# Ajax0564/VyomAI

Hardware: AMD Instinct MI355X
Metric: training tokens/sec (12L d=768 seq=512 GPT-style decoder, CLM) (higher is better)
Workload: dtype bf16; 1 GPU; configs[1]: GPT-style Decoder 12L d=768 h=12 RoPE vocab 50265, CLM training B=32/GPU seq=512, AdamW, bf16 kernels + fp32 masters; global_batch=32, seq_len=512, parallelism=dp1, attention=none, weights=deterministic recipe (vyomai_amd.recipe)

## Files before the change

### include/vyom_hip.h

```cpp
#ifndef VYOM_HIP_H
#define VYOM_HIP_H

#include <stdint.h>

#ifdef __cplusplus
extern "C" {
#endif

typedef enum { VY_F32 = 0, VY_BF16 = 1 } vy_dtype;

typedef enum {
  VY_OK = 0,
  VY_ERR_ARG = -1,
  VY_ERR_UNSUPPORTED = -2,
  VY_ERR_LAUNCH = -3
} vy_status;

typedef enum {
  VY_ACT_NONE = 0, VY_ACT_GELU_ERF = 1, VY_ACT_GELU_TANH = 2,
  VY_ACT_SILU = 3, VY_ACT_TANH = 4, VY_ACT_SIGMOID = 5, VY_ACT_RELU6 = 6, VY_ACT_LEAKY_RELU = 7
} vy_act;
#define VY_ACT_SAVE_DERIV 0x100

enum {
// ... 71 lines not shown
int vy_gated_act_fwd(const void* gate_up, int64_t ldg, void* out, int64_t ldo, int64_t M, int64_t I,
                     int act, int dtype, void* stream);

int vy_rmsnorm_bwd(const void* dy, int64_t lddy, const void* x, int64_t ldx, const void* w,
                   const void* add_to, int64_t ldadd, void* dx, int64_t lddx, float* dw, float beta,
                   float* ws, int64_t M, int64_t N, float eps, float w_offset, int dtype, void* stream);

int vy_gated_act_bwd(const void* d_act, int64_t lddo, const void* gate_up, int64_t ldg, void* d_gate_up,
                     int64_t lddg, int64_t M, int64_t I, int act, int dtype, void* stream);

int vy_rope_fwd(void* x, int64_t sb, int64_t sh, int64_t sl, const float* cos_tab,
                const float* sin_tab, int64_t pos0, int64_t B, int heads, int64_t L, int dh,
                int inverse, int dtype, void* stream);


int vy_linear_dgrad(const void* dy, int64_t lddy, const void* wt, int64_t ldwt, const void* pre,
                    int64_t ldpre, int act, const void* add_to, int64_t ldadd, const void* add_to2,
                    int64_t ldadd2, void* dx, int64_t lddx, int64_t M, int64_t N, int64_t K, int dtype,
                    void* stream);

int vy_linear_wgrad(const void* dy, int64_t lddy, const void* x, int64_t ldx, float* dw,
                    int64_t lddw, float* db, float beta, const float* alpha_dev, int64_t M, int64_t N,
                    int64_t K, int dtype, void* stream);

typedef struct vy_wgrad_desc {
  const void* dy; int64_t lddy;
  const void* x; int64_t ldx;
  float* dw; int64_t lddw;
  float* db;
  int64_t M, N, K;
} vy_wgrad_desc;
int vy_linear_wgrad_grouped(const vy_wgrad_desc* descs, int32_t n, int dtype, void* stream);

typedef struct vy_colsum_desc {
  float* ws; int32_t W, N;
  float* out0; float* out1;
  int32_t acc;
} vy_colsum_desc;
int vy_linear_wgrad_grouped_cs(const vy_wgrad_desc* descs, int32_t n, const vy_colsum_desc* cs, int32_t ncs, int dtype,
                               void* stream);

int64_t vy_layernorm_bwd_ws_rows(int64_t M);
int vy_layernorm_bwd(const void* dy, int64_t lddy, const void* x, int64_t ldx, const void* gamma,
                     const float* mean, const float* rstd, void* dx, int64_t lddx, float* dgamma,
                     float* dbeta, float beta, float* ws, int64_t M, int64_t N, int dtype,
                     void* stream);
// ... 26 lines not shown
                  float grad_scale, const float* grad_scale_dev, void* stream);
int vy_adamw_step_gated(float* p, const float* g, float* m, float* v, void* p_bf16, int64_t n, float lr,
                        float beta1, float beta2, float eps, float weight_decay, int64_t step,
                        float grad_scale, const float* grad_scale_dev, const float* gate, void* stream);

int vy_sumsq(const float* x, int64_t n, float* out, float* ws, void* stream);

int vy_linear_dropout_fwd(const void* x, int64_t ldx, const void* w, int64_t ldw, const void* bias,
                          const void* residual, int64_t ldr, void* y, int64_t ldy, int64_t M, int64_t N,
                          int64_t K, float p_drop, uint64_t seed, uint64_t offset, int dtype, void* stream);
int vy_dropout(const void* x, int64_t ldx, void* y, int64_t ldy, int64_t M, int64_t N, float p_drop,
               uint64_t seed, uint64_t offset, int dtype, void* stream);

int vy_act_bwd(const void* dy, int64_t lddy, const void* pre, int64_t ldpre, void* dx, int64_t lddx,
               int64_t M, int64_t N, int act, int dtype, void* stream);

int vy_xent_fwd(const void* logits, int64_t ld, const int64_t* labels, int64_t ignore_index, float* lse,
                float* loss_sum, float* count, int64_t M, int64_t V, int32_t* err_flag, int dtype, void* stream);
int vy_xent_bwd(void* logits, int64_t ld, const int64_t* labels, int64_t ignore_index, const float* lse,
                const float* gscale, const float* count, int64_t M, int64_t V, int dtype, void* stream);
int vy_xent_fused(void* logits, int64_t ld, const int64_t* labels, int64_t ignore_index, float* lse,
                  float* loss_sum, const float* count, const float* gscale, int64_t M, int64_t V,
                  int32_t* err_flag, int dtype, void* stream);
int vy_xent_sample_fwd(const void* logits, int64_t ld, const int64_t* labels, int64_t ignore_index, float* lse,
                       float* loss_sum, float* count, int64_t* sampled, float inv_temperature, uint64_t seed,
                       uint64_t offset, int64_t M, int64_t V, int32_t* err_flag, int dtype, void* stream);
int vy_xent_sample_fused(void* logits, int64_t ld, const int64_t* labels, int64_t ignore_index, float* lse,
                         float* loss_sum, const float* count, const float* gscale, int64_t* sampled,
                         float inv_temperature, uint64_t seed, uint64_t offset, int64_t M, int64_t V,
                         int32_t* err_flag, int dtype, void* stream);
int vy_gumbel_noise(float* out, int64_t ld, int64_t M, int64_t V, uint64_t seed, uint64_t offset, void* stream);

int vy_bce_head_fwd(const void* h, int64_t ldh, const void* w, const void* b, float* z, const float* target,
                    const uint8_t* live, float* loss_sum, int64_t M, int64_t d, int dtype, void* stream);
int vy_bce_head_bwd(const void* h, int64_t ldh, const void* w, const float* z, const float* target,
                    const uint8_t* live, const float* gscale, const float* count, void* dh, int64_t lddh, float* dw,
                    float* db, int accumulate, int64_t M, int64_t d, int dtype, void* stream);

int vy_mlm_mask(const int64_t* ids, int64_t n, const int64_t* special_ids, int32_t n_special, float fraction,
                int64_t mask_id, int64_t vocab, int64_t ignore_index, uint64_t seed, uint64_t offset,
                int64_t* masked_ids, int64_t* labels, uint8_t* masked, void* stream);


int vy_logprob_fwd(const void* logits, int64_t ld, const int64_t* labels, const float* weight, float* lse,
                   float* logp, int64_t M, int64_t V, int32_t* err_flag, int dtype, void* stream);
int vy_logprob_bwd(void* logits, int64_t ld, const int64_t* labels, const float* weight, const float* lse,
// ... 81 lines not shown
```

### vyomai_amd/_lib.py

```python
from __future__ import annotations

import ctypes as C
import os
from typing import Optional

_HERE = os.path.dirname(os.path.abspath(__file__))
LIB_PATH = os.environ.get("VY_LIB_PATH") or os.path.join(_HERE, "lib", "libvyom_hip.so")

VY_F32, VY_BF16 = 0, 1
ACT_NONE, ACT_GELU_ERF, ACT_GELU_TANH = 0, 1, 2
ACT_SILU, ACT_TANH, ACT_SIGMOID, ACT_RELU6, ACT_LEAKY_RELU = 3, 4, 5, 6, 7
ACT_SAVE_DERIV = 0x100
MASK_NONE, MASK_CAUSAL, MASK_KEYPAD, MASK_ADDITIVE = 0, 1, 2, 4

_p, _i64, _i, _f, _u64 = C.c_void_p, C.c_int64, C.c_int, C.c_float, C.c_uint64

PROTOTYPES = {
    "vy_linear_fwd": [_p, _i64, _p, _i64, _p, _p, _i64, _p, _i64, _p, _i64, _i64, _i64, _i, _i, _p],
    "vy_qkv_rope_fwd": [_p, _i64, _p, _i64, _p, _p, _p, _i64,
                        _p, _i64, _i64, _i64, _p, _i64, _i64, _i64, _p, _i64, _i64, _i64,
                        _i64, _i64, _i64, _i, _i, _i, _i, _p],
    "vy_attn_fwd": [_p, _i64, _i64, _i64, _p, _i64, _i64, _i64, _p, _i64, _i64, _i64,
                    _p, _i64, _i64, _p, _i, _i64, _p, _i64, _p, _i64, _i64,
                    _i64, _i, _i, _i64, _i64, _i, _f, _i, _p],
    "vy_attn_decode": [_p, _i64, _i64, _p, _i64, _i64, _i64, _p, _i64, _i64, _i64,
                       _p, _i64, _i64, _i, _i, _i64, _i, _f, _i, _p],
    "vy_paged_rope_write": [_p, _i64, _p, _p, _p, _p, _i64, _p, _p, _i64, _i, _i64, _i, _i, _i, _i, _p],
    "vy_paged_qknorm_rope_write": [_p, _i64, _p, _p, _p, _p, _i64, _p, _p, _f, _p, _p, _i64, _i, _i64, _i, _i, _i, _i,
                                   _p],
    "vy_attn_paged_decode": [_p, _i64, _p, _p, _p, _i64, _i, _p, _i64, _p, _i64, _p, _i64, _i64, _i, _i, _i, _f, _i,
                             _p, _i64, _i, _p],
    "vy_attn_paged_prefill": [_p, _i64, _p, _p, _i64, _i, _p, _i64, _p, _p, _i64, _i64, _i64, _p, _i64, _i, _i, _i, _f,
                              _i, _p],
    "vy_paged_gather": [_p, _p, _i64, _i, _p, _i64, _i64, _p, _p, _i, _i, _i, _p],
    "vy_layernorm_fwd": [_p, _i64, _p, _p, _p, _i64, _p, _p, _i64, _i64, _f, _i, _p],
    "vy_rmsnorm_fwd": [_p, _i64, _p, _p, _i64, _i64, _i64, _f, _f, _i, _p],
    "vy_gated_act_fwd": [_p, _i64, _p, _i64, _i64, _i64, _i, _i, _p],
    "vy_rmsnorm_bwd": [_p, _i64, _p, _i64, _p, _p, _i64, _p, _i64, _p, _f, _p, _i64, _i64, _f, _f, _i, _p],
    "vy_gated_act_bwd": [_p, _i64, _p, _i64, _p, _i64, _i64, _i64, _i, _i, _p],
    "vy_rope_fwd": [_p, _i64, _i64, _i64, _p, _p, _i64, _i64, _i, _i64, _i, _i, _i, _p],
    "vy_linear_dgrad": [_p, _i64, _p, _i64, _p, _i64, _i, _p, _i64, _p, _i64, _p, _i64, _i64, _i64, _i64, _i, _p],
    "vy_linear_wgrad": [_p, _i64, _p, _i64, _p, _i64, _p, _f, _p, _i64, _i64, _i64, _i, _p],
    "vy_linear_wgrad_grouped": [_p, _i, _i, _p],
    "vy_linear_wgrad_grouped_cs": [_p, _i, _p, _i, _i, _p],
    "vy_layernorm_bwd_partial": [_p, _i64, _p, _i64, _p, _p, _p, _p, _i64, _p, _i64, _i64, _i, _p],
    "vy_layernorm_bwd": [_p, _i64, _p, _i64, _p, _p, _p, _p, _i64, _p, _p, _f, _p, _i64, _i64, _i, _p],
    "vy_attn_bwd": [_p, _i64, _i64, _i64, _p, _i64, _i64, _i64, _p, _i64, _i64, _i64,
                    _p, _p, _i64, _i64, _p, _p,
                    _p, _i64, _i64, _i64, _p, _i64, _i64, _i64, _p, _i64, _i64, _i64,
                    _i, _i64, _p, _i64, _p, _p, _i64, _i64, _i, _i, _i64, _i64, _i, _f, _i, _p],
    "vy_adamw_step": [_p, _p, _p, _p, _p, _i64, _f, _f, _f, _f, _f, _i64, _f, _p, _p],
    "vy_adamw_step_gated": [_p, _p, _p, _p, _p, _i64, _f, _f, _f, _f, _f, _i64, _f, _p, _p, _p],
    "vy_sumsq": [_p, _i64, _p, _p, _p],
    "vy_linear_dropout_fwd": [_p, _i64, _p, _i64, _p, _p, _i64, _p, _i64, _i64, _i64, _i64, _f, _u64, _u64, _i, _p],
    "vy_dropout": [_p, _i64, _p, _i64, _i64, _i64, _f, _u64, _u64, _i, _p],
    "vy_act_bwd": [_p, _i64, _p, _i64, _p, _i64, _i64, _i64, _i, _i, _p],
    "vy_xent_fwd": [_p, _i64, _p, _i64, _p, _p, _p, _i64, _i64, _p, _i, _p],
    "vy_xent_bwd": [_p, _i64, _p, _i64, _p, _p, _p, _i64, _i64, _i, _p],
    "vy_xent_fused": [_p, _i64, _p, _i64, _p, _p, _p, _p, _i64, _i64, _p, _i, _p],
    "vy_xent_sample_fwd": [_p, _i64, _p, _i64, _p, _p, _p, _p, _f, _u64, _u64, _i64, _i64, _p, _i, _p],
    "vy_xent_sample_fused": [_p, _i64, _p, _i64, _p, _p, _p, _p, _p, _f, _u64, _u64, _i64, _i64, _p, _i, _p],
    "vy_gumbel_noise": [_p, _i64, _i64, _i64, _u64, _u64, _p],
    "vy_bce_head_fwd": [_p, _i64, _p, _p, _p, _p, _p, _p, _i64, _i64, _i, _p],
    "vy_bce_head_bwd": [_p, _i64, _p, _p, _p, _p, _p, _p, _p, _i64, _p, _p, _i, _i64, _i64, _i, _p],
    "vy_mlm_mask": [_p, _i64, _p, _i, _f, _i64, _i64, _i64, _u64, _u64, _p, _p, _p, _p],
    "vy_logprob_fwd": [_p, _i64, _p, _p, _p, _p, _i64, _i64, _p, _i, _p],
    "vy_logprob_bwd": [_p, _i64, _p, _p, _p, _i64, _i64, _i, _p],
    "vy_logprob_fused": [_p, _i64, _p, _p, _p, _p, _i64, _i64, _p, _i, _p],
    "vy_transpose_batched": [_p, _i, _i, _i, _p],
    "vy_embedding_fwd": [_p, _i64, _p, _p, _i64, _i64, _i64, _i64, _p, _i, _p],
    "vy_embedding_bwd": [_p, _i64, _p, _p, _i64, _i64, _i64, _i64, _i64, _i, _p],
    "vy_transpose": [_p, _i64, _p, _i64, _i64, _i64, _i, _p],
    "vy_greedy_step": [_p, _i64, _i64, _i64, _i, _p, _i64, _i64, _p, _i64, _p, _i, _p, _p, _p],
    "vy_sampling_probs": [_p, _i64, _i64, _i64, _i, _f, _i, _f, _p, _i64, _p],
    "vy_sample_rows": [_p, _i64, _i64, _i64, _i, _p, _p, _p, _p, _p, _p, _p],
    "vy_decoder_step": [_p, _p, _i64, _p, _p, _p, _i64, _p],
    "vy_gemma_decoder_step": [_p, _p, _i64, _p, _i64, _p],
    "vy_cast": [_p, _p, _i64, _i, _i, _p],
    "vy_ddp_unique_id": [_p],
    "vy_ddp_init": [_p, _i, _i],
    "vy_ddp_all_reduce_async": [_p, _i64, _i, _p],
    "vy_ddp_destroy": [],
# ... 67 lines not shown
```

### vyomai_amd/autograd_train.py

```python
from __future__ import annotations

import os

import weakref
from typing import Optional

import torch

from . import _lib, ops
from ._lib import ACT_GELU_ERF, ACT_NONE, VyomHipError
from .layers.attention import _shadow
from .layers.mask import AttnMask
from .layers.positional_embeddings import resolve_freqs

BF16 = torch.bfloat16


WEIGHT_EPOCH = [0]


class _WtRegistry:

    def __init__(self) -> None:
        self.entries = []
# ... 523 lines not shown
    logits = buf[:, :V]
    ops.linear(n.view(buf.shape[0], -1), _shadow(w, dt), None if bias is None else _shadow(bias, dt), out=logits)
    return buf, logits


def _rehome(x, ld, dtype, reuse=False):
    V = x.shape[-1]
    if reuse and x.stride(-1) == 1 and x.stride(-2) == ld and x.dtype == dtype:
        buf = torch.as_strided(x, (*x.shape[:-1], ld), x.stride())
        if ld != V:
            buf[..., V:].zero_()
        return buf
    buf = torch.zeros((*x.shape[:-1], ld), dtype=dtype, device=x.device)
    buf[..., :V] = x
    return buf


def _shifted_labels(labels, ignore_index, dev):
    shifted = torch.full(labels.shape, ignore_index, dtype=torch.long, device=dev)
    shifted[:, :-1] = labels[:, 1:]
    return shifted.view(-1)


def _xent_forward(logits, shifted, ignore_index, err_flag=None, in_place=True, sample=None):
    V = logits.shape[1]
    dev = logits.device
    lse = torch.empty(logits.shape[0], dtype=torch.float32, device=dev)
    acc = torch.zeros(2, dtype=torch.float32, device=dev)
    fused = in_place and V <= 65536 and logits.dtype == BF16
    if fused:
        acc[1] = ((shifted != ignore_index) & (shifted >= 0) & (shifted < V)).sum()
        if sample is None:
            ops.xent_fused_(logits, shifted, ignore_index, lse, acc[0:1], acc[1:2], _one(dev), err_flag)
        else:
            ops.xent_sample_fused_(logits, shifted, ignore_index, lse, acc[0:1], acc[1:2], _one(dev), *sample, err_flag)
    elif sample is None:
        ops.xent_fwd(logits, shifted, ignore_index, lse, acc[0:1], acc[1:2], err_flag)
    else:
        ops.xent_sample_fwd(logits, shifted, ignore_index, lse, acc[0:1], acc[1:2], *sample, err_flag)
    return acc[0] / acc[1].clamp_min(1.0), lse, acc, fused


def _xent_backward(logits, shifted, ignore_index, lse, acc, fused, gout):
    gs = gout.detach().to(torch.float32).reshape(1).contiguous()
    if fused:
        return gs
    ops.xent_bwd_(logits, shifted, ignore_index, lse, gs, acc[1:2])
    return None


class LMHeadFn(torch.autograd.Function):

    @staticmethod
    def forward(ctx, hidden, wd, bd, ln_w, ln_b, wv, bias, eps):
        _require_bf16(hidden)
        dt = hidden.dtype
        pre, g, n, mean, rstd = _head_transform(hidden, wd, bd, ln_w, ln_b, eps)
        V = wv.shape[0]
        ld = _row_stride(V)
        buf = torch.zeros((*hidden.shape[:-1], ld), dtype=dt, device=hidden.device)
        logits = buf[..., :V]
        ops.linear(n, _shadow(wv, dt), _shadow(bias, dt), out=logits)
        ctx.save_for_backward(hidden, pre, g, n, mean, rstd)
        ctx.params = (wd, bd, ln_w, ln_b, wv, bias)
        ctx.ld = ld
        return logits

    @staticmethod
    def backward(ctx, dlogits):
        hidden, pre, g, n, mean, rstd = ctx.saved_tensors
        wd, bd, ln_w, ln_b, wv, bias = ctx.params
        dt = hidden.dtype
        buf = _rehome(dlogits, ctx.ld, dt, reuse=True)
        dn = ops.linear_dgrad(buf, _wt_padded(wv, dt, ctx.ld))
        dwv, dbias = _wgrad(buf[..., :wv.shape[0]], n, wv, bias)
        return (*_head_transform_backward(dn, hidden, pre, g, mean, rstd, wd, bd, ln_w, ln_b), dwv, dbias, None)


class LMHeadLossFn(torch.autograd.Function):

    @staticmethod
    def forward(ctx, hidden, labels, ignore_index, wd, bd, ln_w, ln_b, wv, bias, eps, err_flag=None, shift=True,
                sample=None):
        _require_bf16(hidden)
        pre, g, n, mean, rstd = _head_transform(hidden, wd, bd, ln_w, ln_b, eps)
        buf, logits = _vocab_logits(n, wv, bias)
        dev = hidden.device
        shifted = _shifted_labels(labels, ignore_index, dev) if shift else labels.to(dev).reshape(-1).contiguous()
        sampled = None
        if sample is not None:
            sampled = torch.empty(shifted.shape, dtype=torch.long, device=dev)
            sample = (sampled, *sample)
        loss, lse, acc, fused = _xent_forward(logits, shifted, ignore_index, err_flag, sample=sample)
        ctx.save_for_backward(hidden, pre, g, n, mean, rstd, buf, shifted, lse, acc)
        ctx.params = (wd, bd, ln_w, ln_b, wv, bias)
        ctx.ignore = ignore_index
        ctx.fused = fused
        if sampled is None:
            return loss
        sampled = sampled.view(labels.shape)
        ctx.mark_non_differentiable(sampled)
        return loss, sampled

    @staticmethod
    def backward(ctx, gout, *_):
        hidden, pre, g, n, mean, rstd, buf, shifted, lse, acc = ctx.saved_tensors
        wd, bd, ln_w, ln_b, wv, bias = ctx.params
        dt = hidden.dtype
        logits = buf[:, :wv.shape[0]]
        alpha = _xent_backward(logits, shifted, ctx.ignore, lse, acc, ctx.fused, gout)
        dn = ops.linear_dgrad(buf, _wt_padded(wv, dt, buf.shape[1]))
        if alpha is not None:
            dn = dn * alpha.to(dt)
        dwv, dbias = _wgrad(logits, n.view(buf.shape[0], -1), wv, bias, alpha=alpha)
        dh, dwd, dbd, dgam, dbet = _head_transform_backward(dn.view(g.shape), hidden, pre, g, mean, rstd, wd, bd, ln_w, ln_b)
        return dh, None, None, dwd, dbd, dgam, dbet, dwv, dbias, None, None, None, None
# ... 256 lines not shown
        ctx.save_for_backward(n)
        ctx.meta = (table, table_pending, ld)
        return logits

    @staticmethod
    def backward(ctx, dlogits):
        (n,) = ctx.saved_tensors
        table, table_pending, ld = ctx.meta
        V = table.shape[0]
        buf = _rehome(dlogits.reshape(-1, V), ld, n.dtype)
        dn, dtab = _tied_head_backward(buf, V, n, table, table_pending, None)
        return dn, dtab, None


class ShiftedXentFn(torch.autograd.Function):

    @staticmethod
    def forward(ctx, logits, labels, ignore_index):
        _require_bf16(logits)
        B, L, V = logits.shape
        if logits.stride(-1) != 1 or logits.stride(1) % 8 or logits.stride(0) != L * logits.stride(1):
            logits = _rehome(logits, _row_stride(V), logits.dtype)[..., :V]
        l2 = torch.as_strided(logits, (B * L, V), (logits.stride(1), 1), logits.storage_offset())
        shifted = _shifted_labels(labels, ignore_index, logits.device)
        loss, lse, acc, _ = _xent_forward(l2, shifted, ignore_index, in_place=False)
        ctx.save_for_backward(l2, shifted, lse, acc)
        ctx.meta = (ignore_index, (B, L, V))
        return loss

    @staticmethod
    def backward(ctx, gout):
        l2, shifted, lse, acc = ctx.saved_tensors
        ignore_index, shape = ctx.meta
        ld = l2.stride(0)
        buf = torch.empty((l2.shape[0], ld), dtype=l2.dtype, device=l2.device)
        d2 = buf[:, :l2.shape[1]]
        d2.copy_(l2)
        _xent_backward(d2, shifted, ignore_index, lse, acc, False, gout)
        return torch.as_strided(buf, shape, (shape[1] * ld, ld, 1)), None, None


class TiedLMHeadLossFn(torch.autograd.Function):

    @staticmethod
    def forward(ctx, hidden, labels, ignore_index, ln_w, eps, table, table_pending, err_flag=None):
        _require_bf16(hidden)
        n = ops.rmsnorm(hidden, _shadow(ln_w, hidden.dtype), eps, 0.0)
        buf, logits = _vocab_logits(n, table, None)
        shifted = _shifted_labels(labels, ignore_index, hidden.device)
        loss, lse, acc, fused = _xent_forward(logits, shifted, ignore_index, err_flag)
        ctx.save_for_backward(hidden, n, buf, shifted, lse, acc)
        ctx.meta = (ln_w, eps, table, table_pending, ignore_index, fused)
        return loss

    @staticmethod
    def backward(ctx, gout):
        hidden, n, buf, shifted, lse, acc = ctx.saved_tensors
        ln_w, eps, table, table_pending, ignore_index, fused = ctx.meta
        V = table.shape[0]
        alpha = _xent_backward(buf[:, :V], shifted, ignore_index, lse, acc, fused, gout)
        dn, dtab = _tied_head_backward(buf, V, n, table, table_pending, alpha)
        dh, dlnw = _rms_bwd(dn, hidden, ln_w, eps)
        return dh, None, None, dlnw, None, dtab, None, None


def logprob_rows(input_ids, selection_mask):
    B, L = input_ids.shape
    labels = torch.zeros((B, L), dtype=torch.long, device=input_ids.device)
    labels[:, :-1] = input_ids[:, 1:]
    m = selection_mask.to(device=input_ids.device, dtype=torch.float32)
    w = torch.zeros((B, L), dtype=torch.float32, device=input_ids.device)
    w[:, :-1] = m[:, 1:]
    total = w.sum(-1, keepdim=True)
# ... 41 lines not shown
```

### vyomai_amd/csrc/vy_bwd.hip

```cpp
#include "vy_attn_tile.h"
#include <float.h>
#include <stdlib.h>
#include <string.h>

namespace {


__device__ __forceinline__ int xcd_remap(int bid, int nwg) {
  const int xcd = bid & 7, q = nwg >> 3, r = nwg & 7;
  return (xcd < r ? xcd * (q + 1) : r * (q + 1) + (xcd - r) * q) + (bid >> 3);
}

__device__ __forceinline__ bf16x8 tr_pair(const char* base, int row_bytes) {
  const s16x4 lo = __builtin_amdgcn_ds_read_tr16_b64_v4i16((VY_LDS s16x4*)(base));
  const s16x4 hi = __builtin_amdgcn_ds_read_tr16_b64_v4i16((VY_LDS s16x4*)(base + 8 * row_bytes));
  union { struct { s16x4 a, b; } s; bf16x8 v; } u;
  u.s.a = lo; u.s.b = hi;
  return u.v;
}

typedef __attribute__((ext_vector_type(2))) __bf16 bf16x2_t;

template <int BT, int MS_, bool MF16>
struct WgradTile {
// ... 231 lines not shown
    }
    const bool hi = kq >= 2;
#pragma unroll
    for (int i = 0; i < TI; ++i)
#pragma unroll
      for (int jp = 0; jp < JH; ++jp) {
        const int k = kw + 16 * (2 * jp + (hi ? 1 : 0)) + r16;
#pragma unroll
        for (int r = 0; r < 4; ++r) {
          const unsigned x = __builtin_bit_cast(unsigned, acc[i][2 * jp][r] * alpha);
          const unsigned y = __builtin_bit_cast(unsigned, acc[i][2 * jp + 1][r] * alpha);
          auto sw = __builtin_amdgcn_permlane32_swap(x, y, false, false);
          const int nlo = nw + 16 * i + 4 * (kq & 1) + r;
          if (k < K) {
            if (nlo < N) atomicAdd(dW + (int64_t)nlo * lddw + k, __builtin_bit_cast(float, (unsigned)sw[0]));
            if (nlo + 8 < N) atomicAdd(dW + (int64_t)(nlo + 8) * lddw + k, __builtin_bit_cast(float, (unsigned)sw[1]));
          }
        }
      }
  }
};

template <int BN, int BKW, int MS, int NS, bool MF16>
__device__ __forceinline__ void wgrad_tn_bf16_body(
    const bf16* __restrict__ dY, int64_t lddy, const bf16* __restrict__ X, int64_t ldx,
    float* __restrict__ dW, int64_t lddw, float* __restrict__ db, const float* __restrict__ alpha_dev,
    int M, int N, int K, int tiles_k, int tiles_nk, int m_chunk, int diag, int wg) {
  static_assert(BN == BKW && ((BN == 128 && MS == 64 && NS == 2) || (BN == 256 && MS == 32 && NS == 4)),
                "built shapes: 128 x 128 x 64 in 2 stages, 256 x 256 x 32 in 4");
  typedef WgradTile<BN, MS, MF16> Tile;
  typedef std::conditional_t<MF16, WgradMma16<Tile>, WgradMma32<Tile>> Mma;
  constexpr int STAGE = Tile::STAGE, PS = 2 * Tile::PP;
  __shared__ __attribute__((aligned(16))) char smem[NS * STAGE];
  const int tid = threadIdx.x, lane = tid & 63;
  const int wave = __builtin_amdgcn_readfirstlane(tid >> 6);
  const int wn = wave >> 1, wk = wave & 1;
  const int split = wg / tiles_nk, t2 = wg - split * tiles_nk;
  const int tile_n = t2 / tiles_k, tile_k = t2 - tile_n * tiles_k;
  const int n0 = tile_n * BN, k0 = tile_k * BKW;
  const int m_begin = split * m_chunk;
  const int m_end = min(M, m_begin + m_chunk);
  if (m_begin >= m_end) return;

  Tile t(dY, lddy, X, ldx, n0, k0, N, K, m_begin, m_end, wave, lane);
  const bool do_db = db != nullptr && tile_k == 0 && wk == 0;
  Mma mma(smem, lane, wn, wk);
  const int nst = t.nst;
#pragma unroll
  for (int s_ = 0; s_ < NS - 1; ++s_)
    if (s_ < nst) t.stage(s_, smem + s_ * STAGE);
  for (int s = 0; s < nst; ++s) {
    const int younger = min(NS - 2, nst - 1 - s);
    if (younger >= 2) asm volatile("s_waitcnt vmcnt(%0)" ::"n"(2 * PS) : "memory");
    else if (younger == 1) asm volatile("s_waitcnt vmcnt(%0)" ::"n"(PS) : "memory");
    else asm volatile("s_waitcnt vmcnt(0)" ::: "memory");
    __builtin_amdgcn_s_barrier();
    asm volatile("" ::: "memory");
    if (s + NS - 1 < nst) t.stage(s + NS - 1, smem + (s + NS - 1) % NS * STAGE);
    mma.mma_stage(s % NS * STAGE, do_db);
  }
  if (diag == 1) {
    if (mma.acc[0][0][0] == 12345.678f) dW[0] = 1.f;
    return;
  }
  const float alpha = alpha_dev ? *alpha_dev : 1.0f;
  mma.epilogue(dW, lddw, db, do_db, alpha, n0 + wn * 64, k0 + wk * Tile::WKT, N, K);
}

template <int BN, int BKW, int MS, int NS, bool MF16>
__global__ __launch_bounds__(BN * 2, BN == 128 ? 2 : 1) void wgrad_tn_bf16_kernel(
    const bf16* __restrict__ dY, int64_t lddy, const bf16* __restrict__ X, int64_t ldx,
    float* __restrict__ dW, int64_t lddw, float* __restrict__ db, const float* __restrict__ alpha_dev,
    int M, int N, int K, int tiles_k, int tiles_nk, int m_chunk, int diag) {
  wgrad_tn_bf16_body<BN, BKW, MS, NS, MF16>(dY, lddy, X, ldx, dW, lddw, db, alpha_dev, M, N, K, tiles_k, tiles_nk, m_chunk,
                                            diag, xcd_remap(blockIdx.x, gridDim.x));
}

struct WgradItem {
  const bf16* dY; const bf16* X; float* dW; float* db;
  int64_t lddy, ldx, lddw;
  int M, N, K, tiles_k, tiles_nk, m_chunk, item0;
};
struct WgradGroup { WgradItem g[8]; int n; };

struct ColsumItem { const float* ws; float* out0; float* out1; int W, N, rps, acc, blk0; };
struct ColsumGroup { ColsumItem c[8]; int n; int items; };

__device__ __forceinline__ void colsum_slab_block(const ColsumItem& it, int blk) {
  __shared__ float red[2][2][4][64];
  const int tid = threadIdx.x;
  const int c = tid & 63, g = (tid >> 6) & 3, h = tid >> 8;
  const int n = blk * 64 + c;
  const int W = it.W, N = it.N, rps = it.rps;
  const float* __restrict__ ws = it.ws;
  const bool one = rps >= W;
  float ta = 0.f, tb = 0.f;
  for (int s0 = 0; s0 * rps < W; s0 += 2) {
    const int w0 = (s0 + h) * rps, w1 = min(W, w0 + rps);
// ... 37 lines not shown
__global__ __launch_bounds__(BN * 2, 1) void wgrad_tn_bf16_grouped_kernel(WgradGroup grp, ColsumGroup cs, int diag) {
  if ((int)blockIdx.x >= cs.items) {
    const int blk = (int)blockIdx.x - cs.items;
    int d = 0;
#pragma unroll
    for (int i = 1; i < 8; ++i)
      if (i < cs.n && blk >= cs.c[i].blk0) d = i;
    ColsumItem it = cs.c[0];
#pragma unroll
    for (int i = 1; i < 8; ++i)
      if (d == i) it = cs.c[i];
    colsum_slab_block(it, blk - it.blk0);
    return;
  }
  const int id = xcd_remap(blockIdx.x, cs.items);
  int d = 0;
#pragma unroll
  for (int i = 1; i < 8; ++i)
    if (i < grp.n && id >= grp.g[i].item0) d = i;
  WgradItem it = grp.g[0];
#pragma unroll
  for (int i = 1; i < 8; ++i)
    if (d == i) it = grp.g[i];
  wgrad_tn_bf16_body<BN, BKW, MS, NS, MF16>(it.dY, it.lddy, it.X, it.ldx, it.dW, it.lddw, it.db, nullptr, it.M, it.N, it.K,
                                            it.tiles_k, it.tiles_nk, it.m_chunk, diag, id - it.item0);
}

__global__ __launch_bounds__(64) void colsum_bf16_kernel(const bf16* __restrict__ dY, int64_t lddy,
                                                         float* __restrict__ db, int M, int N) {
  const int c0 = (blockIdx.x * 64 + threadIdx.x) * 8;
  if (c0 >= N) return;
  const int m0 = blockIdx.y * 256, m1 = min(M, m0 + 256);
  float s[8] = {0, 0, 0, 0, 0, 0, 0, 0};
  for (int m = m0; m < m1; ++m) {
    const bf16x8 v = *reinterpret_cast<const bf16x8*>(dY + (int64_t)m * lddy + c0);
#pragma unroll
    for (int e = 0; e < 8; ++e) s[e] += (float)v[e];
  }
#pragma unroll
  for (int e = 0; e < 8; ++e)
    if (c0 + e < N) atomicAdd(db + c0 + e, s[e]);
}

struct BwdParams {
  const bf16* q; int64_t q_sb, q_sh, q_sl;
  const bf16* k; int64_t k_sb, k_sh, k_sl;
  const bf16* v; int64_t v_sb, v_sh, v_sl;
// ... 364 lines not shown
                     (const float*)x, ldx, dw, lddw, db, alpha_dev, (int)M, (int)N, (int)K, tiles_k, tiles, (int)m_chunk);
  VY_CHECK_LAUNCH(who);
  return VY_OK;
}

bool wgrad_bf16_operands_ok(const void* dy, int64_t lddy, const void* x, int64_t ldx, int64_t N, int64_t K) {
  return !(K % 8 || lddy % 8 || ldx % 8 || lddy < vy_cdiv(N, 8) * 8 || (uintptr_t)dy % 16 || (uintptr_t)x % 16);
}

struct WgradSplit { int64_t splits, m_chunk; };
WgradSplit wgrad_split(int64_t M, int64_t want) {
  const int64_t max_splits = vy_cdiv(M, 256);
  if (want > max_splits) want = max_splits;
  if (want < 1) want = 1;
  const int64_t m_chunk = vy_cdiv(vy_cdiv(M, want), 64) * 64;
  return {vy_cdiv(M, m_chunk), m_chunk};
}

int wgrad_env(const char* name, int dflt) { const char* e = getenv(name); return e ? atoi(e) : dflt; }

int wgrad_m16() { static const int v = wgrad_env("VY_WGRAD_M16", 1); return v; }
int wgrad_diag() { static const int v = wgrad_env("VY_WGRAD_DIAG", 0); return v; }

}

extern "C" int vy_linear_wgrad(const void* dy, int64_t lddy, const void* x, int64_t ldx, float* dw,
                               int64_t lddw, float* db, float beta, const float* alpha_dev, int64_t M,
                               int64_t N, int64_t K, int dtype, void* stream) {
  const char* who = "vy_linear_wgrad";
  if (dtype != VY_BF16 && dtype != VY_F32) VY_FAIL(VY_ERR_ARG, "%s: bad dtype %d", who, dtype);
  if (!dy || !x || !dw || M <= 0 || N <= 0 || K <= 0) VY_FAIL(VY_ERR_ARG, "%s: bad arguments", who);
  if (dtype == VY_F32) {
    if (beta != 0.f && beta != 1.f) VY_FAIL(VY_ERR_ARG, "%s: beta must be 0 or 1", who);
    return wgrad_f32(who, dy, lddy, x, ldx, dw, lddw, db, beta, alpha_dev, M, N, K, (hipStream_t)stream);
  }
  if (!wgrad_bf16_operands_ok(dy, lddy, x, ldx, N, K))
    VY_FAIL(VY_ERR_ARG, "%s: K and leading dimensions must be multiples of 8 (lddy >= roundup8(N)), operands 16-byte aligned", who);
  if (beta != 0.f && beta != 1.f) VY_FAIL(VY_ERR_ARG, "%s: beta must be 0 or 1", who);
  static const int wv = wgrad_env("VY_WGRAD_VARIANT", -1);
  static const int tgt = wgrad_env("VY_WGRAD_TARGET", 0);
  if (wv != -1 && wv != 0 && wv != 8)
    VY_FAIL(VY_ERR_UNSUPPORTED, "%s: VY_WGRAD_VARIANT=%d was removed (the values left are 0 and 8; unset selects by shape)", who, wv);
  hipStream_t st = (hipStream_t)stream;
  if (beta == 0.f) {
    if (hipMemset2DAsync(dw, lddw * sizeof(float), 0, K * sizeof(float), N, st) != hipSuccess)
      VY_FAIL(VY_ERR_LAUNCH, "%s: memset failed", who);
    if (db && hipMemsetAsync(db, 0, N * sizeof(float), st) != hipSuccess)
      VY_FAIL(VY_ERR_LAUNCH, "%s: memset failed", who);
  }
  const bool big = wv < 0 ? (N >= 8192 && M >= 4096) : wv == 8;
  const int BT = big ? 256 : 128;
  const int tiles_k = (int)vy_cdiv(K, BT), tiles = (int)vy_cdiv(N, BT) * tiles_k;
  const WgradSplit sp = wgrad_split(M, tgt > 0 ? vy_cdiv(tgt, tiles) : big ? 256 / tiles : vy_cdiv(384, tiles));
  const int w16 = wgrad_m16();
  auto kernel = big ? (w16 ? wgrad_tn_bf16_kernel<256, 256, 32, 4, true> : wgrad_tn_bf16_kernel<256, 256, 32, 4, false>)
                    : (w16 >= 2 ? wgrad_tn_bf16_kernel<128, 128, 64, 2, true> : wgrad_tn_bf16_kernel<128, 128, 64, 2, false>);
  hipLaunchKernelGGL(kernel, dim3((unsigned)(tiles * sp.splits)), dim3(BT * 2), 0, st, (const bf16*)dy, lddy, (const bf16*)x,
                     ldx, dw, lddw, db, alpha_dev, (int)M, (int)N, (int)K, tiles_k, tiles, (int)sp.m_chunk, wgrad_diag());
  VY_CHECK_LAUNCH(who);
  return VY_OK;
}

static int wgrad_grouped(const char* who, const vy_wgrad_desc* descs, int32_t n, const vy_colsum_desc* cs, int32_t ncs,
                        int dtype, void* stream) {
  if (dtype != VY_BF16 && dtype != VY_F32) VY_FAIL(VY_ERR_ARG, "%s: bad dtype %d", who, dtype);
  if (n < 0 || n > 8 || (n > 0 && !descs) || ncs < 0 || ncs > 8 || (ncs > 0 && !cs) || n + ncs == 0)
    VY_FAIL(VY_ERR_ARG, "%s: 1..8 descriptors", who);
  for (int i = 0; i < ncs; ++i)
    if (!cs[i].ws || cs[i].W <= 0 || cs[i].N <= 0 || (cs[i].acc != 0 && cs[i].acc != 1))
      VY_FAIL(VY_ERR_ARG, "%s: column-sum descriptor %d: bad arguments", who, i);
  if (dtype == VY_F32) {
    for (int i = 0; i < ncs; ++i)
      if (int rc = vy_ln_colsum(cs[i].ws, cs[i].W, cs[i].N, cs[i].out0, cs[i].out1, cs[i].acc, (hipStream_t)stream)) return rc;
    for (int i = 0; i < n; ++i) {
      const vy_wgrad_desc& d = descs[i];
      if (!d.dy || !d.x || !d.dw || d.M <= 0 || d.N <= 0 || d.K <= 0) VY_FAIL(VY_ERR_ARG, "%s: descriptor %d: bad arguments", who, i);
      if (int rc = wgrad_f32(who, d.dy, d.lddy, d.x, d.ldx, d.dw, d.lddw, d.db, 1.f, nullptr, d.M, d.N, d.K, (hipStream_t)stream)) return rc;
    }
    return VY_OK;
  }
  int64_t tiles_total = 0;
// ... 580 lines not shown
```

### vyomai_amd/csrc/vy_misc.hip

```cpp
#include "vy_common.h"
#include <stdarg.h>
#include <string.h>

static thread_local char g_err[512] = "";
void vy_set_error(const char* fmt, ...) {
  va_list ap;
  va_start(ap, fmt);
  vsnprintf(g_err, sizeof(g_err), fmt, ap);
  va_end(ap);
}
extern "C" const char* vy_last_error(void) { return g_err; }
extern "C" int vy_abi_version(void) { return 5; }

namespace {

template <typename T, int CH>
__global__ __launch_bounds__(256) void layernorm_fwd_kernel(const T* __restrict__ x, int64_t ldx,
                                                            const T* __restrict__ gamma,
                                                            const T* __restrict__ beta, T* __restrict__ y,
                                                            int64_t ldy, float* __restrict__ mean_out,
                                                            float* __restrict__ rstd_out, int64_t M, int N,
                                                            float eps) {
  constexpr int VEC = Chunk<T>::VEC;
  const int lane = threadIdx.x & 63;
// ... 982 lines not shown
extern "C" int vy_xent_fused(void* logits, int64_t ld, const int64_t* labels, int64_t ignore_index, float* lse,
                             float* loss_sum, const float* count, const float* gscale, int64_t M, int64_t V,
                             int32_t* err_flag, int dtype, void* stream) {
  return row_fused("vy_xent_fused", loss_sum && count && gscale, logits, ld, labels,
                   XentRow<false>{ignore_index, gscale, count, loss_sum, nullptr}, lse, M, V, err_flag, dtype, stream);
}

extern "C" int vy_xent_sample_fwd(const void* logits, int64_t ld, const int64_t* labels, int64_t ignore_index,
                                  float* lse, float* loss_sum, float* count, int64_t* sampled, float inv_temperature,
                                  uint64_t seed, uint64_t offset, int64_t M, int64_t V, int32_t* err_flag, int dtype,
                                  void* stream) {
  XentSampleRow<true> p{{ignore_index, nullptr, nullptr, loss_sum, count}, sampled, inv_temperature, vy_make_noise(seed, offset)};
  return row_lse("vy_xent_sample_fwd", loss_sum && count && sampled, logits, ld, labels, p, lse, M, V, err_flag, dtype, stream);
}

extern "C" int vy_xent_sample_fused(void* logits, int64_t ld, const int64_t* labels, int64_t ignore_index, float* lse,
                                    float* loss_sum, const float* count, const float* gscale, int64_t* sampled,
                                    float inv_temperature, uint64_t seed, uint64_t offset, int64_t M, int64_t V,
                                    int32_t* err_flag, int dtype, void* stream) {
  XentSampleRow<false> p{{ignore_index, gscale, count, loss_sum, nullptr}, sampled, inv_temperature, vy_make_noise(seed, offset)};
  return row_fused("vy_xent_sample_fused", loss_sum && count && gscale && sampled, logits, ld, labels, p, lse, M, V, err_flag, dtype, stream);
}

extern "C" int vy_logprob_fwd(const void* logits, int64_t ld, const int64_t* labels, const float* weight, float* lse,
                              float* logp, int64_t M, int64_t V, int32_t* err_flag, int dtype, void* stream) {
  return row_lse("vy_logprob_fwd", weight && logp, logits, ld, labels, LogprobRow{weight, logp}, lse, M, V, err_flag,
                 dtype, stream);
}

extern "C" int vy_logprob_bwd(void* logits, int64_t ld, const int64_t* labels, const float* weight, const float* lse,
                              int64_t M, int64_t V, int dtype, void* stream) {
  return row_grad("vy_logprob_bwd", weight != nullptr, logits, ld, labels, LogprobRow{weight, nullptr}, lse, M, V, dtype,
                  stream);
}

extern "C" int vy_logprob_fused(void* logits, int64_t ld, const int64_t* labels, const float* weight, float* lse,
                                float* logp, int64_t M, int64_t V, int32_t* err_flag, int dtype, void* stream) {
  return row_fused("vy_logprob_fused", weight && logp, logits, ld, labels, LogprobRow{weight, logp}, lse, M, V,
                   err_flag, dtype, stream);
}

extern "C" int vy_cast(const void* src, void* dst, int64_t n, int src_dtype, int dst_dtype, void* stream) {
  if (!src || !dst || n < 0) VY_FAIL(VY_ERR_ARG, "vy_cast: bad arguments");
  if (n == 0) return VY_OK;
  hipStream_t st = (hipStream_t)stream;
  const int64_t want = vy_cdiv(n, 1024);
// ... 272 lines not shown
```

### vyomai_amd/ops.py

```python
from __future__ import annotations

import math
from typing import NamedTuple, Optional, Tuple

import torch

from . import _lib
from ._lib import call, dtype_code

Tensor = torch.Tensor




class _Lanes:
    active = False
    side: Optional[torch.cuda.Stream] = None
    fork_ev: Optional[torch.cuda.Event] = None
    join_ev: Optional[torch.cuda.Event] = None
    B = L = B0 = 0
    dirty = False
    keep: list = []
    streams = {}

# ... 465 lines not shown
    call("vy_cast", src.data_ptr(), dst.data_ptr(), src.numel(), dtype_code(src.dtype), dtype_code(dst.dtype), _stream())
    return dst


def act_bwd(dy: Tensor, pre: Tensor, act: int) -> Tensor:
    _need_gpu(dy, pre)
    d2, p2 = _rows(dy), _rows(pre)
    M, N = p2.shape
    out = torch.empty((M, N), dtype=dy.dtype, device=dy.device)
    call("vy_act_bwd", d2.data_ptr(), d2.stride(0), p2.data_ptr(), p2.stride(0), out.data_ptr(), out.stride(0),
         M, N, act, dtype_code(dy.dtype), _stream())
    return out.view(pre.shape)


def _row_args(logits2d: Tensor, labels: Tensor, *rows: Tensor, scalars=()) -> None:
    M = logits2d.shape[0]
    assert labels.dtype == torch.long and labels.numel() == M and labels.is_contiguous()
    for t in rows:
        assert t.dtype == torch.float32 and t.numel() == M and t.is_contiguous()
    for t in scalars:
        assert t.dtype == torch.float32 and t.numel() == 1


def xent_fwd(logits2d: Tensor, labels: Tensor, ignore_index: int, lse: Tensor, loss_sum: Tensor, count: Tensor,
             err_flag: Optional[Tensor] = None) -> None:
    _need_gpu(logits2d, labels, lse, loss_sum, count, err_flag)
    _row_args(logits2d, labels, lse, scalars=(loss_sum, count))
    M, V = logits2d.shape
    call("vy_xent_fwd", logits2d.data_ptr(), logits2d.stride(0), labels.data_ptr(), ignore_index, lse.data_ptr(),
         loss_sum.data_ptr(), count.data_ptr(), M, V, _ptr(err_flag), dtype_code(logits2d.dtype), _stream())


def xent_bwd_(logits2d: Tensor, labels: Tensor, ignore_index: int, lse: Tensor, gscale: Tensor, count: Tensor) -> None:
    _need_gpu(logits2d, labels, lse, gscale, count)
    _row_args(logits2d, labels, lse, scalars=(gscale, count))
    M, V = logits2d.shape
    call("vy_xent_bwd", logits2d.data_ptr(), logits2d.stride(0), labels.data_ptr(), ignore_index, lse.data_ptr(),
         gscale.data_ptr(), count.data_ptr(), M, V, dtype_code(logits2d.dtype), _stream())


def xent_fused_(logits2d: Tensor, labels: Tensor, ignore_index: int, lse: Tensor, loss_sum: Tensor,
                count: Tensor, gscale: Tensor, err_flag: Optional[Tensor] = None) -> None:
    _need_gpu(logits2d, labels, lse, loss_sum, count, gscale, err_flag)
    _row_args(logits2d, labels, lse, scalars=(loss_sum, count, gscale))
    M, V = logits2d.shape
    call("vy_xent_fused", logits2d.data_ptr(), logits2d.stride(0), labels.data_ptr(), ignore_index, lse.data_ptr(),
# ... 355 lines not shown
```

Measured before the change: 877,800 tokens/s.

## Balance big wgrad tiles across CUs and fuse label shift/count into one kernel

For the 256-tile wgrad path, the launch now sizes its grid to the number of CUs. Each workgroup walks a contiguous range of (tile, M-slab) work items, crossing tile boundaries with a barrier in between. This is meant to remove tail imbalance when the tile-by-split count does not divide evenly across CUs. Separately, the cross-entropy label shift and valid-label count, previously several small torch ops, become a single one-block kernel that writes the shifted labels and the accumulator, cutting launch overhead. Risks: extra dW read-modify-write passes for split tiles, and a serial one-block kernel for large B*L.

```diff
diff --git a/include/vyom_hip.h b/include/vyom_hip.h
--- a/include/vyom_hip.h
+++ b/include/vyom_hip.h
@@ -117,6 +117,7 @@
 int vy_linear_wgrad(const void* dy, int64_t lddy, const void* x, int64_t ldx, float* dw,
                     int64_t lddw, float* db, float beta, const float* alpha_dev, int64_t M, int64_t N,
                     int64_t K, int dtype, void* stream);
+int vy_debug_set_wgrad_balance(int wgs);
 
 typedef struct vy_wgrad_desc {
   const void* dy; int64_t lddy;
@@ -189,6 +190,8 @@
 int vy_xent_fused(void* logits, int64_t ld, const int64_t* labels, int64_t ignore_index, float* lse,
                   float* loss_sum, const float* count, const float* gscale, int64_t M, int64_t V,
                   int32_t* err_flag, int dtype, void* stream);
+int vy_xent_labels(const int64_t* labels, int64_t ldl, int64_t* out, float* acc, int64_t B, int64_t L, int shift,
+                   int64_t ignore_index, int64_t V, void* stream);
 int vy_xent_sample_fwd(const void* logits, int64_t ld, const int64_t* labels, int64_t ignore_index, float* lse,
                        float* loss_sum, float* count, int64_t* sampled, float inv_temperature, uint64_t seed,
                        uint64_t offset, int64_t M, int64_t V, int32_t* err_flag, int dtype, void* stream);
diff --git a/vyomai_amd/_lib.py b/vyomai_amd/_lib.py
--- a/vyomai_amd/_lib.py
+++ b/vyomai_amd/_lib.py
@@ -41,6 +41,7 @@
     "vy_rope_fwd": [_p, _i64, _i64, _i64, _p, _p, _i64, _i64, _i, _i64, _i, _i, _i, _p],
     "vy_linear_dgrad": [_p, _i64, _p, _i64, _p, _i64, _i, _p, _i64, _p, _i64, _p, _i64, _i64, _i64, _i64, _i, _p],
     "vy_linear_wgrad": [_p, _i64, _p, _i64, _p, _i64, _p, _f, _p, _i64, _i64, _i64, _i, _p],
+    "vy_debug_set_wgrad_balance": [_i],
     "vy_linear_wgrad_grouped": [_p, _i, _i, _p],
     "vy_linear_wgrad_grouped_cs": [_p, _i, _p, _i, _i, _p],
     "vy_layernorm_bwd_partial": [_p, _i64, _p, _i64, _p, _p, _p, _p, _i64, _p, _i64, _i64, _i, _p],
@@ -58,6 +59,7 @@
     "vy_xent_fwd": [_p, _i64, _p, _i64, _p, _p, _p, _i64, _i64, _p, _i, _p],
     "vy_xent_bwd": [_p, _i64, _p, _i64, _p, _p, _p, _i64, _i64, _i, _p],
     "vy_xent_fused": [_p, _i64, _p, _i64, _p, _p, _p, _p, _i64, _i64, _p, _i, _p],
+    "vy_xent_labels": [_p, _i64, _p, _p, _i64, _i64, _i, _i64, _i64, _p],
     "vy_xent_sample_fwd": [_p, _i64, _p, _i64, _p, _p, _p, _p, _f, _u64, _u64, _i64, _i64, _p, _i, _p],
     "vy_xent_sample_fused": [_p, _i64, _p, _i64, _p, _p, _p, _p, _p, _f, _u64, _u64, _i64, _i64, _p, _i, _p],
     "vy_gumbel_noise": [_p, _i64, _i64, _i64, _u64, _u64, _p],
diff --git a/vyomai_amd/autograd_train.py b/vyomai_amd/autograd_train.py
--- a/vyomai_amd/autograd_train.py
+++ b/vyomai_amd/autograd_train.py
@@ -569,14 +569,28 @@
     return shifted.view(-1)
 
 
-def _xent_forward(logits, shifted, ignore_index, err_flag=None, in_place=True, sample=None):
+_XENT_LABELS_KERNEL = os.environ.get("VY_XENT_LABELS", "1") != "0"
+
+
+def _xent_labels(labels, ignore_index, dev, shift, V):
+    if (_XENT_LABELS_KERNEL and labels.dim() == 2 and labels.dtype == torch.long and labels.device == dev
+            and labels.numel() > 0 and (labels.shape[1] == 1 or labels.stride(1) == 1)
+            and (labels.shape[0] == 1 or labels.stride(0) >= labels.shape[1])):
+        return ops.xent_labels(labels, ignore_index, shift, V)
+    flat = _shifted_labels(labels, ignore_index, dev) if shift else labels.to(dev).reshape(-1).contiguous()
+    acc = torch.zeros(2, dtype=torch.float32, device=dev)
+    if V:
+        acc[1] = ((flat != ignore_index) & (flat >= 0) & (flat < V)).sum()
+    return flat, acc
+
+
+def _xent_forward(logits, labels, ignore_index, err_flag=None, in_place=True, sample=None, shift=True):
     V = logits.shape[1]
     dev = logits.device
     lse = torch.empty(logits.shape[0], dtype=torch.float32, device=dev)
-    acc = torch.zeros(2, dtype=torch.float32, device=dev)
     fused = in_place and V <= 65536 and logits.dtype == BF16
+    shifted, acc = _xent_labels(labels, ignore_index, dev, shift, V if fused else 0)
     if fused:
-        acc[1] = ((shifted != ignore_index) & (shifted >= 0) & (shifted < V)).sum()
         if sample is None:
             ops.xent_fused_(logits, shifted, ignore_index, lse, acc[0:1], acc[1:2], _one(dev), err_flag)
         else:
@@ -585,7 +599,7 @@
         ops.xent_fwd(logits, shifted, ignore_index, lse, acc[0:1], acc[1:2], err_flag)
     else:
         ops.xent_sample_fwd(logits, shifted, ignore_index, lse, acc[0:1], acc[1:2], *sample, err_flag)
-    return acc[0] / acc[1].clamp_min(1.0), lse, acc, fused
+    return acc[0] / acc[1].clamp_min(1.0), lse, acc, fused, shifted
 
 
 def _xent_backward(logits, shifted, ignore_index, lse, acc, fused, gout):
@@ -632,13 +646,11 @@
         _require_bf16(hidden)
         pre, g, n, mean, rstd = _head_transform(hidden, wd, bd, ln_w, ln_b, eps)
         buf, logits = _vocab_logits(n, wv, bias)
-        dev = hidden.device
-        shifted = _shifted_labels(labels, ignore_index, dev) if shift else labels.to(dev).reshape(-1).contiguous()
         sampled = None
         if sample is not None:
-            sampled = torch.empty(shifted.shape, dtype=torch.long, device=dev)
+            sampled = torch.empty(labels.numel(), dtype=torch.long, device=hidden.device)
             sample = (sampled, *sample)
-        loss, lse, acc, fused = _xent_forward(logits, shifted, ignore_index, err_flag, sample=sample)
+        loss, lse, acc, fused, shifted = _xent_forward(logits, labels, ignore_index, err_flag, sample=sample, shift=shift)
         ctx.save_for_backward(hidden, pre, g, n, mean, rstd, buf, shifted, lse, acc)
         ctx.params = (wd, bd, ln_w, ln_b, wv, bias)
         ctx.ignore = ignore_index
@@ -941,8 +953,7 @@
         if logits.stride(-1) != 1 or logits.stride(1) % 8 or logits.stride(0) != L * logits.stride(1):
             logits = _rehome(logits, _row_stride(V), logits.dtype)[..., :V]
         l2 = torch.as_strided(logits, (B * L, V), (logits.stride(1), 1), logits.storage_offset())
-        shifted = _shifted_labels(labels, ignore_index, logits.device)
-        loss, lse, acc, _ = _xent_forward(l2, shifted, ignore_index, in_place=False)
+        loss, lse, acc, _, shifted = _xent_forward(l2, labels, ignore_index, in_place=False)
         ctx.save_for_backward(l2, shifted, lse, acc)
         ctx.meta = (ignore_index, (B, L, V))
         return loss
@@ -966,8 +977,7 @@
         _require_bf16(hidden)
         n = ops.rmsnorm(hidden, _shadow(ln_w, hidden.dtype), eps, 0.0)
         buf, logits = _vocab_logits(n, table, None)
-        shifted = _shifted_labels(labels, ignore_index, hidden.device)
-        loss, lse, acc, fused = _xent_forward(logits, shifted, ignore_index, err_flag)
+        loss, lse, acc, fused, shifted = _xent_forward(logits, labels, ignore_index, err_flag)
         ctx.save_for_backward(hidden, n, buf, shifted, lse, acc)
         ctx.meta = (ln_w, eps, table, table_pending, ignore_index, fused)
         return loss
diff --git a/vyomai_amd/csrc/vy_bwd.hip b/vyomai_amd/csrc/vy_bwd.hip
--- a/vyomai_amd/csrc/vy_bwd.hip
+++ b/vyomai_amd/csrc/vy_bwd.hip
@@ -277,25 +277,20 @@
 };
 
 template <int BN, int BKW, int MS, int NS, bool MF16>
-__device__ __forceinline__ void wgrad_tn_bf16_body(
-    const bf16* __restrict__ dY, int64_t lddy, const bf16* __restrict__ X, int64_t ldx,
+__device__ __forceinline__ void wgrad_tn_bf16_piece(
+    char* smem, const bf16* __restrict__ dY, int64_t lddy, const bf16* __restrict__ X, int64_t ldx,
     float* __restrict__ dW, int64_t lddw, float* __restrict__ db, const float* __restrict__ alpha_dev,
-    int M, int N, int K, int tiles_k, int tiles_nk, int m_chunk, int diag, int wg) {
+    int N, int K, int tiles_k, int t2, int m_begin, int m_end, int diag) {
   static_assert(BN == BKW && ((BN == 128 && MS == 64 && NS == 2) || (BN == 256 && MS == 32 && NS == 4)),
                 "built shapes: 128 x 128 x 64 in 2 stages, 256 x 256 x 32 in 4");
   typedef WgradTile<BN, MS, MF16> Tile;
   typedef std::conditional_t<MF16, WgradMma16<Tile>, WgradMma32<Tile>> Mma;
   constexpr int STAGE = Tile::STAGE, PS = 2 * Tile::PP;
-  __shared__ __attribute__((aligned(16))) char smem[NS * STAGE];
   const int tid = threadIdx.x, lane = tid & 63;
   const int wave = __builtin_amdgcn_readfirstlane(tid >> 6);
   const int wn = wave >> 1, wk = wave & 1;
-  const int split = wg / tiles_nk, t2 = wg - split * tiles_nk;
   const int tile_n = t2 / tiles_k, tile_k = t2 - tile_n * tiles_k;
   const int n0 = tile_n * BN, k0 = tile_k * BKW;
-  const int m_begin = split * m_chunk;
-  const int m_end = min(M, m_begin + m_chunk);
-  if (m_begin >= m_end) return;
 
   Tile t(dY, lddy, X, ldx, n0, k0, N, K, m_begin, m_end, wave, lane);
   const bool do_db = db != nullptr && tile_k == 0 && wk == 0;
@@ -322,13 +317,59 @@
   mma.epilogue(dW, lddw, db, do_db, alpha, n0 + wn * 64, k0 + wk * Tile::WKT, N, K);
 }
 
+template <int BN, int MS, int NS, bool MF16>
+constexpr int wgrad_lds_bytes() { return NS * WgradTile<BN, MS, MF16>::STAGE; }
+
+template <int BN, int BKW, int MS, int NS, bool MF16>
+__device__ __forceinline__ void wgrad_tn_bf16_body(
+    char* smem, const bf16* __restrict__ dY, int64_t lddy, const bf16* __restrict__ X, int64_t ldx,
+    float* __restrict__ dW, int64_t lddw, float* __restrict__ db, const float* __restrict__ alpha_dev,
+    int M, int N, int K, int tiles_k, int tiles_nk, int m_chunk, int diag, int wg) {
+  const int split = wg / tiles_nk, t2 = wg - split * tiles_nk;
+  const int m_begin = split * m_chunk;
+  const int m_end = min(M, m_begin + m_chunk);
+  if (m_begin >= m_end) return;
+  wgrad_tn_bf16_piece<BN, BKW, MS, NS, MF16>(smem, dY, lddy, X, ldx, dW, lddw, db, alpha_dev, N, K, tiles_k, t2, m_begin, m_end,
+                                             diag);
+}
+
+template <int BN, int BKW, int MS, int NS, bool MF16>
+__device__ __forceinline__ void wgrad_tn_bf16_ranges(
+    char* smem, const bf16* __restrict__ dY, int64_t lddy, const bf16* __restrict__ X, int64_t ldx,
+    float* __restrict__ dW, int64_t lddw, float* __restrict__ db, const float* __restrict__ alpha_dev,
+    int M, int N, int K, int tiles_k, int tiles_nk, int q, int diag, int w) {
+  const int nst = (M + MS - 1) / MS;
+  int i = w * q;
+  const int end = min(tiles_nk * nst, i + q);
+  for (bool first = true; i < end; first = false) {
+    const int t2 = i / nst, s0 = i - t2 * nst, s1 = min(nst, s0 + (end - i));
+    if (!first) {
+      asm volatile("s_waitcnt vmcnt(0)" ::: "memory");
+      __builtin_amdgcn_s_barrier();
+      asm volatile("" ::: "memory");
+    }
+    wgrad_tn_bf16_piece<BN, BKW, MS, NS, MF16>(smem, dY, lddy, X, ldx, dW, lddw, db, alpha_dev, N, K, tiles_k, t2, s0 * MS,
+                                               min(M, s1 * MS), diag);
+    i += s1 - s0;
+  }
+}
+
 template <int BN, int BKW, int MS, int NS, bool MF16>
 __global__ __launch_bounds__(BN * 2, BN == 128 ? 2 : 1) void wgrad_tn_bf16_kernel(
     const bf16* __restrict__ dY, int64_t lddy, const bf16* __restrict__ X, int64_t ldx,
     float* __restrict__ dW, int64_t lddw, float* __restrict__ db, const float* __restrict__ alpha_dev,
-    int M, int N, int K, int tiles_k, int tiles_nk, int m_chunk, int diag) {
-  wgrad_tn_bf16_body<BN, BKW, MS, NS, MF16>(dY, lddy, X, ldx, dW, lddw, db, alpha_dev, M, N, K, tiles_k, tiles_nk, m_chunk,
-                                            diag, xcd_remap(blockIdx.x, gridDim.x));
+    int M, int N, int K, int tiles_k, int tiles_nk, int m_chunk, int diag, int bal_q) {
+  __shared__ __attribute__((aligned(16))) char smem[wgrad_lds_bytes<BN, MS, NS, MF16>()];
+  const int wg = xcd_remap(blockIdx.x, gridDim.x);
+  if constexpr (BN == 256) {
+    if (bal_q > 0) {
+      wgrad_tn_bf16_ranges<BN, BKW, MS, NS, MF16>(smem, dY, lddy, X, ldx, dW, lddw, db, alpha_dev, M, N, K, tiles_k, tiles_nk,
+                                                  bal_q, diag, wg);
+      return;
+    }
+  }
+  wgrad_tn_bf16_body<BN, BKW, MS, NS, MF16>(smem, dY, lddy, X, ldx, dW, lddw, db, alpha_dev, M, N, K, tiles_k, tiles_nk,
+                                            m_chunk, diag, wg);
 }
 
 struct WgradItem {
@@ -412,7 +453,8 @@
 #pragma unroll
   for (int i = 1; i < 8; ++i)
     if (d == i) it = grp.g[i];
-  wgrad_tn_bf16_body<BN, BKW, MS, NS, MF16>(it.dY, it.lddy, it.X, it.ldx, it.dW, it.lddw, it.db, nullptr, it.M, it.N, it.K,
+  __shared__ __attribute__((aligned(16))) char smem[wgrad_lds_bytes<BN, MS, NS, MF16>()];
+  wgrad_tn_bf16_body<BN, BKW, MS, NS, MF16>(smem, it.dY, it.lddy, it.X, it.ldx, it.dW, it.lddw, it.db, nullptr, it.M, it.N, it.K,
                                             it.tiles_k, it.tiles_nk, it.m_chunk, diag, id - it.item0);
 }
 
@@ -823,7 +865,22 @@
 int wgrad_m16() { static const int v = wgrad_env("VY_WGRAD_M16", 1); return v; }
 int wgrad_diag() { static const int v = wgrad_env("VY_WGRAD_DIAG", 0); return v; }
 
-}
+int g_wgrad_balance = -2;
+int wgrad_balance() {
+  if (g_wgrad_balance == -2) g_wgrad_balance = wgrad_env("VY_WGRAD_BALANCE", -1);
+  if (g_wgrad_balance >= 0) return g_wgrad_balance;
+  static int cus[64];
+  int dev = 0, n = 0;
+  if (hipGetDevice(&dev) != hipSuccess || dev < 0) return 0;
+  if (dev < 64 && cus[dev]) return cus[dev];
+  if (hipDeviceGetAttribute(&n, hipDeviceAttributeMultiprocessorCount, dev) != hipSuccess || n < 1) return 0;
+  if (dev < 64) cus[dev] = n;
+  return n;
+}
+
+}
+
+extern "C" int vy_debug_set_wgrad_balance(int wgs) { g_wgrad_balance = wgs < 0 ? -1 : wgs; return 0; }
 
 extern "C" int vy_linear_wgrad(const void* dy, int64_t lddy, const void* x, int64_t ldx, float* dw,
                                int64_t lddw, float* db, float beta, const float* alpha_dev, int64_t M,
@@ -853,11 +910,17 @@
   const int BT = big ? 256 : 128;
   const int tiles_k = (int)vy_cdiv(K, BT), tiles = (int)vy_cdiv(N, BT) * tiles_k;
   const WgradSplit sp = wgrad_split(M, tgt > 0 ? vy_cdiv(tgt, tiles) : big ? 256 / tiles : vy_cdiv(384, tiles));
+  int64_t grid = tiles * sp.splits, bal_q = 0;
+  if (big && tgt <= 0) {
+    const int64_t W = wgrad_balance(), nst = vy_cdiv(M, 32), total = tiles * nst;
+    const int64_t q = W > 0 ? vy_cdiv(total, W) : 0;
+    if (q >= nst && total + q < INT32_MAX) grid = vy_cdiv(total, q), bal_q = q;
+  }
   const int w16 = wgrad_m16();
   auto kernel = big ? (w16 ? wgrad_tn_bf16_kernel<256, 256, 32, 4, true> : wgrad_tn_bf16_kernel<256, 256, 32, 4, false>)
                     : (w16 >= 2 ? wgrad_tn_bf16_kernel<128, 128, 64, 2, true> : wgrad_tn_bf16_kernel<128, 128, 64, 2, false>);
-  hipLaunchKernelGGL(kernel, dim3((unsigned)(tiles * sp.splits)), dim3(BT * 2), 0, st, (const bf16*)dy, lddy, (const bf16*)x,
-                     ldx, dw, lddw, db, alpha_dev, (int)M, (int)N, (int)K, tiles_k, tiles, (int)sp.m_chunk, wgrad_diag());
+  hipLaunchKernelGGL(kernel, dim3((unsigned)grid), dim3(BT * 2), 0, st, (const bf16*)dy, lddy, (const bf16*)x, ldx, dw, lddw,
+                     db, alpha_dev, (int)M, (int)N, (int)K, tiles_k, tiles, (int)sp.m_chunk, wgrad_diag(), (int)bal_q);
   VY_CHECK_LAUNCH(who);
   return VY_OK;
 }
diff --git a/vyomai_amd/csrc/vy_misc.hip b/vyomai_amd/csrc/vy_misc.hip
--- a/vyomai_amd/csrc/vy_misc.hip
+++ b/vyomai_amd/csrc/vy_misc.hip
@@ -1028,6 +1028,50 @@
   return row_fused("vy_xent_sample_fused", loss_sum && count && gscale && sampled, logits, ld, labels, p, lse, M, V, err_flag, dtype, stream);
 }
 
+namespace {
+__global__ __launch_bounds__(1024) void xent_labels_kernel(const int64_t* __restrict__ labels, int64_t ldl,
+                                                           int64_t* __restrict__ out, float* __restrict__ acc, int64_t B,
+                                                           int64_t L, int shift, int64_t ignore_index, int64_t V) {
+  __shared__ int part[16];
+  const int tid = threadIdx.x;
+  const int n = (int)(B * L), Li = (int)L;
+  const int db = 1024 / Li, dt = 1024 - db * Li;
+  int b = tid / Li, t = tid - b * Li;
+  int cnt = 0;
+#pragma unroll 8
+  for (int i = tid; i < n; i += 1024) {
+    const int64_t v = (shift && t == Li - 1) ? ignore_index : labels[b * ldl + t + shift];
+    out[i] = v;
+    cnt += (v != ignore_index && v >= 0 && v < V) ? 1 : 0;
+    b += db, t += dt;
+    if (t >= Li) t -= Li, ++b;
+  }
+#pragma unroll
+  for (int o = 32; o > 0; o >>= 1) cnt += __shfl_xor(cnt, o, 64);
+  if ((tid & 63) == 0) part[tid >> 6] = cnt;
+  __syncthreads();
+  if (tid == 0) {
+    int total = 0;
+#pragma unroll
+    for (int w = 0; w < 16; ++w) total += part[w];
+    acc[0] = 0.f;
+    acc[1] = (float)total;
+  }
+}
+}
+
+extern "C" int vy_xent_labels(const int64_t* labels, int64_t ldl, int64_t* out, float* acc, int64_t B, int64_t L,
+                              int shift, int64_t ignore_index, int64_t V, void* stream) {
+  if (!labels || !out || !acc || B <= 0 || L <= 0 || ldl < L || (shift != 0 && shift != 1))
+    VY_FAIL(VY_ERR_ARG, "vy_xent_labels: bad arguments");
+  const int64_t lim = (int64_t)1 << 24;
+  if (B >= lim || L >= lim || B * L >= lim) VY_FAIL(VY_ERR_UNSUPPORTED, "vy_xent_labels: B * L must stay below 2^24 (the count is a float)");
+  hipLaunchKernelGGL(xent_labels_kernel, dim3(1), dim3(1024), 0, (hipStream_t)stream, labels, ldl, out, acc, B, L, shift,
+                     ignore_index, V);
+  VY_CHECK_LAUNCH("vy_xent_labels");
+  return VY_OK;
+}
+
 extern "C" int vy_logprob_fwd(const void* logits, int64_t ld, const int64_t* labels, const float* weight, float* lse,
                               float* logp, int64_t M, int64_t V, int32_t* err_flag, int dtype, void* stream) {
   return row_lse("vy_logprob_fwd", weight && logp, logits, ld, labels, LogprobRow{weight, logp}, lse, M, V, err_flag,
diff --git a/vyomai_amd/ops.py b/vyomai_amd/ops.py
--- a/vyomai_amd/ops.py
+++ b/vyomai_amd/ops.py
@@ -511,6 +511,20 @@
         assert t.dtype == torch.float32 and t.numel() == 1
 
 
+def xent_labels(labels: Tensor, ignore_index: int, shift: bool, V: int) -> Tuple[Tensor, Tensor]:
+    _need_gpu(labels)
+    assert labels.dtype == torch.long and labels.dim() == 2 and labels.numel() > 0
+    B, L = labels.shape
+    assert L == 1 or labels.stride(1) == 1
+    ldl = labels.stride(0) if B > 1 else L
+    assert ldl >= L
+    out = torch.empty(B * L, dtype=torch.long, device=labels.device)
+    acc = torch.empty(2, dtype=torch.float32, device=labels.device)
+    call("vy_xent_labels", labels.data_ptr(), ldl, out.data_ptr(), acc.data_ptr(), B, L, int(bool(shift)), ignore_index, V,
+         _stream())
+    return out, acc
+
+
 def xent_fwd(logits2d: Tensor, labels: Tensor, ignore_index: int, lse: Tensor, loss_sum: Tensor, count: Tensor,
              err_flag: Optional[Tensor] = None) -> None:
     _need_gpu(logits2d, labels, lse, loss_sum, count, err_flag)
```

Measured after the change: 868,000 tokens/s. 1.1% lower.
